# kfjahnke/envutil

Hardware: AMD Instinct MI355X
Metric: Mpix/s reprojected (16K lat/lon->cubemap, b-spline-3) (higher is better)
Workload: dtype f32

## Files before the change

envutil_amd/csrc/eu_render4.hip:

```cpp
#include <cstdio>
#include <cstring>
#include <vector>
#include <algorithm>
#include "eu_packed_dev.h"
#include "eu_launch.h"

#define EU4_TW 16
#define EU4_TH 8
#define EU4_WAVES 4
#ifndef EU4_WAVES0
#define EU4_WAVES0 1
#define EU4_TEXELS 384
#define EU4_OCC0 4
#endif
#define EU4_UNIT_ROWS 4
#define EU4_COL_FLOATS 8
#define EU4_MAX_PLANS 16

__device__ __forceinline__ void eu4_box_reduce(int &mn0, int &mn1, int &mx0, int &mx1)
{
#define EU4_RED(ctrl)                                        \
  "v_min_i32_dpp %0, %0, %0 " ctrl "\n\t"                    \
  "v_min_i32_dpp %1, %1, %1 " ctrl "\n\t"                    \
  "v_max_i32_dpp %2, %2, %2 " ctrl "\n\t"                    \
// ... 31 lines not shown
struct eu4_plan {
  const float *atab_g;
  const int *tileplan;
  const float *coltab;
  int tiles16;
  const int *l2_rows;
  int l2_off[9];
  int l2_half;
  unsigned long long l2_magic;
  const int *l1_ent;
  int l1_off[9];
  int l1_ecols;
  unsigned long long l1_magic;
  const int *xtab;
  const int *boxtab;
#ifdef EU5_STAMPS
  unsigned long long *stamps;
#endif
};

#ifdef EU5_STAMPS
#define EU5_STAMP(k) do { asm volatile("" ::: "memory"); st_[k] = __builtin_amdgcn_s_memtime(); asm volatile("" ::: "memory"); } while (0)
#define EU5_STAMP32(k) do { asm volatile("" ::: "memory"); st_[k] = (unsigned)__builtin_amdgcn_s_memtime(); asm volatile("" ::: "memory"); } while (0)
#else
#define EU5_STAMP(k) do { } while (0)
#define EU5_STAMP32(k) do { } while (0)
#endif

template <int NCH, int DEG, int PRJ>
__device__ __forceinline__ void eu4_tile(const eu_render_params &p, const eu4_plan &w, const float *atab,
// ... 272 lines not shown
  __syncthreads();
  if (threadIdx.x == 0) { listed = 0; last = atomicAdd(p.wl + EU4_WL_DONE1, 1) == (int)gridDim.x - 1; }
  __syncthreads();
  if (last) {
    int mine = 0;
    for (int i = threadIdx.x; i < EU4_SHARDS; i += 256)
      mine += __hip_atomic_load(p.wl + EU4_WL_SHARD(i), __ATOMIC_RELAXED, __HIP_MEMORY_SCOPE_AGENT);
    atomicAdd(&listed, mine);
    for (int i = threadIdx.x; i <= EU4_SHARDS + 8; i += 256)
      __hip_atomic_store(p.wl + 16 * i, 0, __ATOMIC_RELAXED, __HIP_MEMORY_SCOPE_AGENT);
    __syncthreads();
    if (threadIdx.x == 0) __hip_atomic_store(p.wl + EU4_WL_LISTED, listed, __ATOMIC_RELAXED, __HIP_MEMORY_SCOPE_AGENT);
  }
}

static long long eu4_followers_plan = 0, eu4_followers_last = 0;
extern "C" unsigned long long eu_hip_share_follower_tiles(void) { return (unsigned long long)eu4_followers_last; }
static int eu4_boxtab_last = 0;
static long long eu4_boxtab_tiles_last = 0;
extern "C" int eu_hip_boxtab_used(void) { return eu4_boxtab_last; }
extern "C" unsigned long long eu_hip_boxtab_tiles(void) { return (unsigned long long)eu4_boxtab_tiles_last; }

#ifndef EU4_DIRECT_WGS
#define EU4_DIRECT_WGS 2048
#endif

template <int NCH, int DEG, int PRJ>
static int launch4_ndp(const eu_render_params &p, const eu4_plan &w, hipStream_t st)
{
  if constexpr (PRJ == EU_SPHERICAL) {
    static const int cus = [] {
      int dev = 0, n = 0;
      if (hipGetDevice(&dev) != hipSuccess) return 0;
      if (hipDeviceGetAttribute(&n, hipDeviceAttributeMultiprocessorCount, dev) != hipSuccess) return 0;
      return n;
    }();
    const bool fast = eu_staged_fast_profile(p);
    const bool bt = fast && w.boxtab != nullptr && p.out_stride < (1ll << 25);
    int per_cu = 0;
    if (bt) {
      static const int occ = [] { int n = 0; return hipOccupancyMaxActiveBlocksPerMultiprocessor(&n, eu_render5_kernel<NCH, DEG, PRJ, true, true>, 64 * EU5_WAVES, 0) == hipSuccess ? n : 0; }();
      per_cu = occ;
    } else if (fast) {
      static const int occ = [] { int n = 0; return hipOccupancyMaxActiveBlocksPerMultiprocessor(&n, eu_render5_kernel<NCH, DEG, PRJ, true>, 64 * EU5_WAVES, 0) == hipSuccess ? n : 0; }();
      per_cu = occ;
    } else {
      static const int occ = [] { int n = 0; return hipOccupancyMaxActiveBlocksPerMultiprocessor(&n, eu_render5_kernel<NCH, DEG, PRJ, false>, 64 * EU5_WAVES, 0) == hipSuccess ? n : 0; }();
      per_cu = occ;
    }
    const int wgs = (cus / 8) * 8 * per_cu;
    if (wgs <= 0) return -1;
    if (fast) eu4_followers_last = eu4_followers_plan;
    eu4_boxtab_last = bt;
    if (bt) hipLaunchKernelGGL((eu_render5_kernel<NCH, DEG, PRJ, true, true>), dim3((unsigned)wgs), dim3(64 * EU5_WAVES), 0, st, p, w);
    else if (fast) hipLaunchKernelGGL((eu_render5_kernel<NCH, DEG, PRJ, true>), dim3((unsigned)wgs), dim3(64 * EU5_WAVES), 0, st, p, w);
    else hipLaunchKernelGGL((eu_render5_kernel<NCH, DEG, PRJ, false>), dim3((unsigned)wgs), dim3(64 * EU5_WAVES), 0, st, p, w);
  } else {
    const int units = (p.tiles_y + EU4_UNIT_ROWS - 1) / EU4_UNIT_ROWS;
    dim3 grid((unsigned)(8 * ((w.tiles16 + EU4_WAVES0 - 1) / EU4_WAVES0)), (unsigned)EU4_UNIT_ROWS, (unsigned)((units + 7) / 8));
    hipLaunchKernelGGL((eu_render4s_kernel<NCH, DEG, PRJ>), grid, dim3(64 * EU4_WAVES0), 0, st, p, w);
  }
  if (hipGetLastError() != hipSuccess) return -1;
  hipLaunchKernelGGL((eu_render4d_kernel<NCH, DEG, PRJ>), dim3(EU4_DIRECT_WGS), dim3(256), 0, st, p, w);
  if (hipGetLastError() != hipSuccess) {
    (void)hipMemsetAsync(p.wl, 0, EU4_WL_ENTRIES * sizeof(int), st);
    return -1;
  }
  return 0;
}

template <int NCH, int DEG>
static int launch4_nd(const eu_render_params &p, const eu4_plan &w, hipStream_t st)
{
  switch (p.src.prj) {
    case EU_SPHERICAL: return launch4_ndp<NCH, DEG, EU_SPHERICAL>(p, w, st);
    case EU_CUBEMAP: return launch4_ndp<NCH, DEG, EU_CUBEMAP>(p, w, st);
    case EU_BIATAN6: return launch4_ndp<NCH, DEG, EU_BIATAN6>(p, w, st);
// ... 15 lines not shown
static_assert(EU_STAGED_TILE_ROWS == EU4_TH && EU_STAGED_MAX_TILES_Y == 65535 * 8 * EU4_UNIT_ROWS, "eu_select.h: eu_staged_covers");
namespace {
struct plan_cache {
  std::vector<unsigned char> key;
  eu_dev_buf<int> tileplan, l2_rows, l1_ent, xtab, boxtab;
  bool has_boxtab = false;
  long long boxtab_tiles = 0;
  eu_dev_buf<float> coltab;
  float *atab = nullptr;
  int planned_rows = 0;
  int l2_off[9] = {};
  int l1_off[9] = {};
  int l1_ecols = 1;
  long long follower_tiles = 0;
  hipStream_t last_stream = nullptr;
} g4s[EU_MAX_SLOTS];
#define g4 (g4s[eu_current_slot()])

bool ensure_atab()
{
  if (g4.atab) return true;
  std::vector<float> tab(768, 0.0f);
  for (int i = 0; i < EU_ATAN_TAB_ENTRIES; i++) eu_atan_tab_entry(i, tab.data() + 8 * i);
  if (hipMalloc((void **)&g4.atab, tab.size() * sizeof(float)) != hipSuccess) return false;
  return hipMemcpy(g4.atab, tab.data(), tab.size() * sizeof(float), hipMemcpyHostToDevice) == hipSuccess;
}

template <int DEG>
void launch_colplan(const eu_render_params &p, float *ct, const float *k, hipStream_t st)
{
// ... 50 lines not shown
      for (size_t j = 0; j < plans.size() / 4 && id < 0; j++)
        if (memcmp(&plans[4 * j], k, sizeof k) == 0) id = (int)j;
      if (id < 0 && plans.size() / 4 < EU4_MAX_PLANS) {
        id = (int)(plans.size() / 4);
        plans.insert(plans.end(), k, k + 4);
      }
      tp[(size_t)ty] = id;
    }
  }
  const int nplans = (int)(plans.size() / 4);
  if (g4.tileplan.reserve(tp.size()) != hipSuccess) return -1;
  if (g4.coltab.reserve(std::max<size_t>(1, nplans) * (size_t)p.width * EU4_COL_FLOATS) != hipSuccess) return -1;
  if (hipStreamSynchronize(st) != hipSuccess) return -1;
  if (g4.last_stream && g4.last_stream != st && hipStreamSynchronize(g4.last_stream) != hipSuccess) return -1;
  if (hipMemcpy(g4.tileplan.p, tp.data(), tp.size() * sizeof(int), hipMemcpyHostToDevice) != hipSuccess) return -1;
  g4.planned_rows = 0;
  for (int v : tp) g4.planned_rows += v >= 0;
  auto paired = [&](int m) { return 2 * m + 1 < p.tiles_y && tp[(size_t)2 * m] >= 0 && tp[(size_t)2 * m] == tp[(size_t)2 * m + 1]; };
  {
    std::vector<int> rows[8], all;
    for (int r = 0; r < p.tiles_y; r++)
      if (!paired(r >> 1)) rows[(r / EU5_UNIT_ROWS) & 7].push_back(r);
    for (int x = 0; x < 8; x++) { g4.l2_off[x] = (int)all.size(); all.insert(all.end(), rows[x].begin(), rows[x].end()); }
    g4.l2_off[8] = (int)all.size();
    if (!upload(g4.l2_rows, all, 1)) return -1;
  }
  g4.has_boxtab = false; g4.boxtab_tiles = 0;
  if (sw.boxtab && eu_staged_fast_profile(p)) {
    const long long ntiles = (long long)g4.l2_off[8] * tiles16;
    const long long bytes = ntiles * (EU5_BT_RECS * 16);
    if (bytes <= (long long)sw.boxtab_max_kb * 1024) {
      if (g4.boxtab.reserve((size_t)std::max<long long>(1, ntiles) * (EU5_BT_RECS * 4)) != hipSuccess) return -1;
      if (ntiles > 0) {
        switch (p.src.degree) {
          case 1: launch_boxplan<1>(p, g4.atab, g4.l2_rows.p, tiles16, (int)ntiles, g4.boxtab.p, st); break;
          case 2: launch_boxplan<2>(p, g4.atab, g4.l2_rows.p, tiles16, (int)ntiles, g4.boxtab.p, st); break;
          default: launch_boxplan<3>(p, g4.atab, g4.l2_rows.p, tiles16, (int)ntiles, g4.boxtab.p, st); break;
        }
        if (hipGetLastError() != hipSuccess) return -1;
      }
// ... 37 lines not shown

void eu4_fill_plan(eu4_plan &w)
{
  w.tileplan = g4.tileplan.p;
  w.coltab = g4.coltab.p;
  w.l2_rows = g4.l2_rows.p;
  for (int x = 0; x < 9; x++) w.l2_off[x] = g4.l2_off[x];
  w.l2_half = (w.tiles16 + 1) / 2;
  w.l2_magic = (1ull << 40) / (unsigned long long)w.l2_half + 1;
  w.l1_ent = g4.l1_ent.p;
  for (int x = 0; x < 9; x++) w.l1_off[x] = g4.l1_off[x];
  w.l1_ecols = g4.l1_ecols;
  w.l1_magic = (1ull << 40) / (unsigned long long)w.l1_ecols + 1;
  w.xtab = g4.xtab.p;
  w.boxtab = g4.has_boxtab ? g4.boxtab.p : nullptr;
}

int launch4(const eu_render_params &p, const eu4_plan &w, hipStream_t st)
{
  switch (p.nch) {
    case 3: return launch4_n<3>(p, w, st);
    case 4: return launch4_n<4>(p, w, st);
  }
  return -2;
}

#ifdef EU5_STAMPS
int launch4_stamped(const eu_render_params &p, eu4_plan &w, hipStream_t st)
{
  static unsigned long long *d_st = nullptr; static size_t st_cap = 0; static int dumps = 0;
// ... 54 lines not shown
  hipStream_t st = (hipStream_t)stream;
  if (!ensure_atab()) return -1;
  w.atab_g = g4.atab;
  if (p.src.prj == EU_SPHERICAL) {
    std::vector<unsigned char> key = eu4_plan_key(p, plan_gen, *sw);
    if (key != g4.key) {
      if (eu4_build_plans(p, w.tiles16, *sw, h_row, h_row_floats, st)) return -1;
      g4.key.swap(key);
    }
    if (sw->r4 != 1 && !eu_staged_worth(p.src.degree, g4.planned_rows, p.tiles_y)) { *launches = 0; return 0; }
  }
  eu4_fill_plan(w);
  eu4_followers_plan = g4.follower_tiles;
  eu4_boxtab_tiles_last = w.boxtab ? g4.boxtab_tiles : 0;
  g4.last_stream = st;
#ifdef EU5_STAMPS
  return launch4_stamped(p, w, st);
#else
  return launch4(p, w, st);
#endif
}
```

envutil_amd/csrc/eu_render5.h:

```cpp
#define EU5_WAVES 4
#ifndef EU5_TEXELS
#define EU5_TEXELS 576
#endif
#ifndef EU5_OCC
#define EU5_OCC 4
#endif
#ifndef EU5_UNIT_ROWS
#define EU5_UNIT_ROWS 4
#endif

typedef const __attribute__((address_space(3))) eu4_f4 *eu5_l4ptr;

template <int NCH, int DEG>
__device__ __forceinline__ void eu5_taps(eu_lptr lt, int a, int b, int pitch, const eu_f2 *wx, const eu_f2 *wy,
                                         eu_f2 tx, eu_f2 ty, eu_f2 &rga, eu_f2 &bxa, eu_f2 &rgb, eu_f2 &bxb)
{
  constexpr int order = DEG + 1;
  if constexpr (DEG == 1) {
    const eu_f2 wl0 = 1.0f - tx, wr0 = tx, wl1 = 1.0f - ty, wr1 = ty;
    const eu4_f4 a00 = *(eu5_l4ptr)(lt + a), a01 = *(eu5_l4ptr)(lt + a + 4);
    const eu4_f4 a10 = *(eu5_l4ptr)(lt + a + pitch), a11 = *(eu5_l4ptr)(lt + a + pitch + 4);
    const eu4_f4 b00 = *(eu5_l4ptr)(lt + b), b01 = *(eu5_l4ptr)(lt + b + 4);
    const eu4_f4 b10 = *(eu5_l4ptr)(lt + b + pitch), b11 = *(eu5_l4ptr)(lt + b + pitch + 4);
    {
// ... 117 lines not shown
  const int y = p.row_begin + tile_y * EU4_TH + rw;
  const int yc = y < p.row_end ? y : p.row_end - 1;
  const float *rt = p.row + (long long)(FAST ? yc : eu_frame_row(yc, p.band_shift, p.band_count, p.band_index)) * EU_ROW_FLOATS;
  const int xa = x0 + 8 * hf + 2 * pr, xb = xa + 1;
  const int xac = xa < p.width ? xa : p.width - 1, xbc = xb < p.width ? xb : p.width - 1;
  T.A0 = rt[0]; T.A1 = rt[1]; T.A2 = rt[2]; T.B0 = rt[3]; T.B1 = rt[4]; T.B2 = rt[5];
  T.c0 = (eu_f2){ p.col[xac], p.col[xbc] };
}

struct eu5_co8 {
  eu_f2 tx, ty;
  int ixa, ixb, iya, iyb;
  eu_i2 ok;
};

template <int DEG>
__device__ __forceinline__ void eu5_coords8(const eu_src_dev &s, const float *atab, const eu5_tab8 &T, eu5_co8 &c)
{
  eu_i2 big0 = { 0, 0 }, big1 = { 0, 0 };
  const eu_f2 c0 = T.c0;
  const eu_f2 rx = T.B0 * c0 + T.A0, ry = T.B1 * c0 + T.A1, rz = T.B2 * c0 + T.A2;
  const eu_i2 ok = { ~eu5_out_of_range3(rx.x, ry.x, rz.x), ~eu5_out_of_range3(rx.y, ry.y, rz.y) };
  const eu_f2 q2 = rx * rx + rz * rz;
  const eu_f2 qs = eu_sqrt2_safe(q2);
  const eu_f2 lat = eu_atan2f_2_lean(ry, qs, atab, 1, big0);
  const eu_f2 lon = eu_atan2f_2_lean(rx, rz, atab, 0, big1);
  c.ok = ok & ~(big0 | big1);
  eu_f2 i0 = { (float)((double)lon.x - s.tex_x0), (float)((double)lon.y - s.tex_x0) };
  if (s.cdiv_ok) i0 = eu_div2_const(i0, s.ext_w, s.rcp_ext_w);
  else i0 = eu_div2_rr(i0, s.ext_w, eu_rcp_refined(s.ext_w));
  i0 = i0 * s.total_w; i0 = i0 - .5f;
  const eu_f2 sx = i0 - s.win_x_off;
  const eu_f2 gx = eu5_gate2(sx, s.gate0, s.lower0, s.upper0);
  eu_f2 fx;
  if constexpr (DEG & 1) fx = (eu_f2){ floorf(gx.x), floorf(gx.y) };
  else fx = (eu_f2){ roundf(gx.x), roundf(gx.y) };
  c.tx = gx - fx;
  c.ixa = (int)fx.x; c.ixb = (int)fx.y;
  eu_f2 i1 = { (float)((double)lat.x - s.tex_y0), (float)((double)lat.y - s.tex_y0) };
  if (s.cdiv_ok) i1 = eu_div2_const(i1, s.ext_h, s.rcp_ext_h);
  else i1 = eu_div2_rr(i1, s.ext_h, eu_rcp_refined(s.ext_h));
  i1 = i1 * s.total_h; i1 = i1 - .5f;
  const eu_f2 sy = i1 - s.win_y_off;
  c.ty = eu5_gate2(sy, s.gate1, s.lower1, s.upper1);
}

template <int DEG>
__device__ __forceinline__ void eu5_split_y(eu5_co8 &c)
{
  const eu_f2 gy = c.ty;
  eu_f2 fy;
  if constexpr (DEG & 1) fy = (eu_f2){ floorf(gy.x), floorf(gy.y) };
  else fy = (eu_f2){ roundf(gy.x), roundf(gy.y) };
  c.ty = gy - fy;
  c.iya = (int)fy.x; c.iyb = (int)fy.y;
}
// ... 401 lines not shown
  if (B.npass == 2) { r[0] = eu5_box_at(B.h0, B.h1, B.h2, B.h3, 31); r[1] = eu5_box_at(B.h0, B.h1, B.h2, B.h3, 63); }
  if (B.npass == 4) {
#pragma unroll
    for (int k = 0; k < 4; k++) r[k] = eu5_box_at(B.q0, B.q1, B.q2, B.q3, 15 + 16 * k);
  }
  int v = 0;
#pragma unroll
  for (int k = 0; k < EU5_BT_RECS; k++) {
#pragma unroll
    for (int i = 0; i < 4; i++)
      if (lane == 4 * k + i) v = eu5_bt_pack(r[k], k == 0 ? cls : 0, i);
  }
  if (lane < 4 * EU5_BT_RECS) tab[(size_t)g * (4 * EU5_BT_RECS) + lane] = v;
}

template <int NCH, int DEG>
__device__ __forceinline__ void eu5_tile_bt(const eu_render_params &p, const eu4_plan &w, const float *atab, float *wtile,
                                            int tile_y, int x0, int lane, const eu5_tab8 &T, eu5_i4 R, eu5_crec rec,
                                            bool have_n, int ty_n, int x0_n, eu5_tab8 &Tn)
{
  constexpr int order = DEG + 1;
  const eu_src_dev &s = p.src;
#ifdef EU5_STAMPS
  unsigned long long st_[8] = { 0, 0, 0, 0, 0, 0, 0, 0 };
#endif
  EU5_STAMP(0);
  const int cls = R.w;
  if (cls & EU5_BT_WORK) {
    if (lane == 0) {
      const int id = tile_y * w.tiles16 + x0 / EU4_TW;
      const int sh = eu4_shard_of(id);
      const int slot = atomicAdd(p.wl + EU4_WL_SHARD(sh), 1);
      p.wl[EU4_WL_ENTRIES + (size_t)slot * EU4_SHARDS + sh] = id;
    }
    if (have_n) eu5_load8<true>(p, ty_n, x0_n, lane, Tn);
    __builtin_amdgcn_s_waitcnt(EU5_WAIT_VM0);
    return;
  }
  const int npass = cls & 7;
  const unsigned lds_tile = (unsigned)(unsigned long long)(eu4_lds_void)wtile;
  eu5_tab8 Tl = T;
  asm volatile("" : "+v"(Tl.c0), "+v"(Tl.A0), "+v"(Tl.A1), "+v"(Tl.A2), "+v"(Tl.B0), "+v"(Tl.B1), "+v"(Tl.B2));
  eu5_box bx = { R.x, R.y, R.x + (R.z & 0xffff), R.y + (R.z >> 16) };
  bool some = npass > 0 && R.z >= 0;
  if (some) eu5_stage<NCH, DEG>(s, bx, lds_tile, lane);
  const int pr = lane & 3, rw = (lane >> 2) & 7, hf = lane >> 5;
  const int y = p.row_begin + tile_y * EU4_TH + rw;
  const bool yin = y < p.row_end;
  const int xa = x0 + 8 * hf + 2 * pr, xb = xa + 1;
  const bool va = yin && xa < p.width, vb = yin && xb < p.width;
  eu_f2 rga = { 0.0f, 0.0f }, bxa = { 0.0f, 0.0f }, rgb = { 0.0f, 0.0f }, bxb = { 0.0f, 0.0f };
  if (npass > 0) {
    eu5_co8 c;
    eu5_coords8<DEG>(s, atab, Tl, c);
    eu5_split_y<DEG>(c);
#ifdef EU5_STAMPS
    asm volatile("" : : "v"(c.iya), "v"(c.iyb), "v"(c.ixa), "v"(c.ixb));
#endif
    EU5_STAMP(2);
#ifdef EU5_STAMPS
    st_[3] = st_[2];
#endif
    eu_f2 wx[order], wy[order];
    if constexpr (DEG >= 2) {
      eu_weights2<DEG>(s.wm, c.ty, wy);
      eu_weights2<DEG>(s.wm, c.tx, wx);
    }
    const int grp = npass == 1 ? 0 : npass == 2 ? hf : (lane >> 4);
#pragma unroll 1
// ... 82 lines not shown
  "v_min_i32_dpp %0, %0, %0 " ctrl "\n\t"                    \
  "v_max_i32_dpp %1, %1, %1 " ctrl "\n\t"                    \
  "s_nop 1\n\t"
  asm("s_nop 1\n\t"
      EU5_RED2("row_shr:1 row_mask:0xf bank_mask:0xf")
      EU5_RED2("row_shr:2 row_mask:0xf bank_mask:0xf")
      EU5_RED2("row_shr:4 row_mask:0xf bank_mask:0xf")
      EU5_RED2("row_shr:8 row_mask:0xf bank_mask:0xf")
      EU5_RED2("row_bcast:15 row_mask:0xa bank_mask:0xf")
      EU5_RED2("row_bcast:31 row_mask:0xc bank_mask:0xf")
      : "+v"(mn), "+v"(mx));
#undef EU5_RED2
  mn = __builtin_amdgcn_readlane(mn, 63); mx = __builtin_amdgcn_readlane(mx, 63);
}

template <int NCH, int DEG>
__device__ __forceinline__ void eu5_group16(const eu_render_params &p, const eu4_plan &w, const float *atab, float *wtile,
                                            eu5_tab16 &T, eu5_cint ent, int n, int m0, int plan0, int tcol, int lane0,
                                            bool have_n, int m_n, int plan_n, int tcol_n)
{
  constexpr int order = DEG + 1;
  const eu_src_dev &s = p.src;
#ifdef EU5_STAMPS
  unsigned st_[8] = { 0, 0, 0, 0, 0, 0, 0, 0 };
#endif
  EU5_STAMP32(0);
  const eu5_cint xt = (eu5_cint)w.xtab;
  int xmn = xt[2 * (plan0 * w.tiles16 + tcol)], xmx = xt[2 * (plan0 * w.tiles16 + tcol) + 1];
  int iyAa, iyAb, iyBa, iyBb, bad, mny = INT_MAX, mxy = INT_MIN;
  eu_f2 tyA, tyB;
  bool off;
// ... 92 lines not shown
      const int oBa = hBa ? ((iyBa - bx.mny) * ibw + (ixa - bx.mnx)) * 4 : 0, oBb = hBb ? ((iyBb - bx.mny) * ibw + (ixb - bx.mnx)) * 4 : 0;
      asm volatile("s_waitcnt vmcnt(0)" ::: "memory");
      __builtin_amdgcn_sched_barrier(0);
      eu5_taps<NCH, DEG>((eu_lptr)wtile, oAa, oAb, ibw * 4, wx, wyA, tx, tyA, rga, bxa, rgb, bxb);
      asm volatile("" : "+v"(rga), "+v"(bxa), "+v"(rgb), "+v"(bxb));
      {
        float qa[4] = { rga.x, rga.y, bxa.x, bxa.y }, qb[4] = { rgb.x, rgb.y, bxb.x, bxb.y };
        float *const orow = p.out + (long long)(ycA - p.row_begin) * p.out_stride;
        if (hAa) eu_put<NCH>(orow, xa, qa);
        if (hAb) eu_put<NCH>(orow, xb, qb);
      }
      __builtin_amdgcn_sched_barrier(0);
      eu5_taps<NCH, DEG>((eu_lptr)wtile, oBa, oBb, ibw * 4, wx, wyB, tx, tyB, rga, bxa, rgb, bxb);
      asm volatile("" : "+v"(rga), "+v"(bxa), "+v"(rgb), "+v"(bxb));
    } else if (mny != INT_MAX) {
      if (lane < 2) {
        const int id = (2 * mk + lane) * w.tiles16 + tc;
        const int sh = eu4_shard_of(id);
        const int slot = atomicAdd(p.wl + EU4_WL_SHARD(sh), 1);
        p.wl[EU4_WL_ENTRIES + (size_t)slot * EU4_SHARDS + sh] = id;
      }
    }
    if (k + 1 < n) {
      const int xa_n = mir_n ? p.width - 1 - (tcol * EU4_TW + xl) : tcol * EU4_TW + xl, xb_n = mir_n ? xa_n - 1 : xa_n + 1;
      const int xac = xa_n < p.width ? xa_n : p.width - 1, xbc = xb_n < p.width ? xb_n : p.width - 1;
      eu5_load_cols(w.coltab + (size_t)plan_k * p.width * EU4_COL_FLOATS, xac, xbc, T);
    } else if (have_n) {
      eu5_load16(p, w.coltab + (size_t)plan_n * p.width * EU4_COL_FLOATS, 2 * m_n, tcol_n * EU4_TW, lane, T);
    }
    __builtin_amdgcn_sched_barrier(0);
    if (fast) {
// ... 41 lines not shown
    const unsigned h = ((unsigned)row() * 0x9E3779B1u) >> 16;
    int c = rx + (int)((h * (unsigned)tiles16) >> 16);
    if (c >= tiles16) c -= tiles16;
    return c;
  }
};

__device__ __forceinline__ int eu5_pair_plan(const int *tileplan, int tiles_y, int m)
{
  if (2 * m + 1 >= tiles_y) return -1;
  const eu5_cint tp = (eu5_cint)tileplan;
  const int a = tp[2 * m], b = tp[2 * m + 1];
  return a == b ? a : -1;
}

template <int NCH, int DEG, int PRJ, bool FAST, bool BOXTAB = false>
__global__ __launch_bounds__(64 * EU5_WAVES, EU5_OCC) void eu_render5_kernel(const eu_render_params p, const eu4_plan w)
{
  __shared__ __attribute__((aligned(16))) float tile_all[EU5_WAVES * EU5_TEXELS * 4];
  __shared__ __attribute__((aligned(16))) float atab[768];
  const int lane0 = threadIdx.x & 63;
  const int wave = __builtin_amdgcn_readfirstlane(threadIdx.x >> 6);
  float *const tile = tile_all + wave * (EU5_TEXELS * 4);
  if (PRJ != EU_CUBEMAP && wave == 0) {
#pragma unroll
    for (int i = 0; i < 3; i++)
      __builtin_amdgcn_global_load_lds((eu4_gbl_void)(w.atab_g + i * 256 + lane0 * 4),
                                       (eu4_lds_void)(atab + i * 256), 16, 0, 0);
    asm volatile("s_waitcnt vmcnt(0)" ::: "memory");
  }
  __syncthreads();
// ... 17 lines not shown
      const unsigned h = ((unsigned)m * 0x9E3779B1u) >> 16;
      int c = pos1 - r * w.l1_ecols + (int)((h * (unsigned)w.l1_ecols) >> 16);
      if (c >= w.l1_ecols) c -= w.l1_ecols;
      tcol = e[1] + c;
      pos1 += K;
      return true;
    };
    eu5_cint e_a = ents, e_n = ents;
    int n_a = 0, m_a = 0, col_a = 0, plan_a = 0, n_n = 0, m_n = 0, col_n = 0, plan_n = 0;
    bool have_a = seek(e_a, n_a, m_a, plan_a, col_a);
    eu5_tab16 T;
    if (have_a) eu5_load16(p, w.coltab + (size_t)plan_a * p.width * EU4_COL_FLOATS, 2 * m_a, col_a * EU4_TW, lane0, T);
#pragma unroll 1
    while (have_a) {
      const bool have_n = seek(e_n, n_n, m_n, plan_n, col_n);
      eu5_group16<NCH, DEG>(p, w, atab, tile, T, e_a, n_a, m_a, plan_a, col_a, lane0, have_n, m_n, have_n ? plan_n : 0, col_n);
      e_a = e_n; n_a = n_n; m_a = m_n; plan_a = plan_n; col_a = col_n; have_a = have_n;
    }
  }
#ifdef EU5_STAMPS
  ws1 = __builtin_amdgcn_s_memtime();
#endif
  eu5_iter<EU5_UNIT_ROWS> it;
  it.xcd = xcd; it.tiles16 = w.tiles16;
  it.units = (p.tiles_y + EU5_UNIT_ROWS - 1) / EU5_UNIT_ROWS;
  it.start(t0, K);
  if constexpr (PAIRS) {
    int *const queue = p.wl + EU4_WL_DYN(xcd);
    const int nbatch = (w.l2_off[xcd + 1] - w.l2_off[xcd]) * w.l2_half;
    const eu5_cint rows2 = (eu5_cint)w.l2_rows + w.l2_off[xcd];
    auto take = [&]() -> int {
      int v = 0;
      if (lane0 == 0) v = atomicAdd(queue, 1);
      return v;
    };
    if constexpr (BOXTAB) {
      static_assert(FAST && PRJ == EU_SPHERICAL, "the box table is that of the FAST lat/lon second loop");
      const eu5_crec bt = (eu5_crec)w.boxtab;
      auto decode = [&](int j, int &ty, int &tcol, int &ti) -> bool {
        if (j >= nbatch) return false;
        const int r = (int)(((unsigned long long)(unsigned)j * w.l2_magic) >> 40);
        ty = rows2[r]; tcol = 2 * (j - r * w.l2_half);
        ti = ((w.l2_off[xcd] + r) * w.tiles16 + tcol) * EU5_BT_RECS;
        return true;
      };
      int ty_a = 0, col_a = 0, ti_a = 0, ty_n = 0, col_n = 0, ti_n = 0;
      bool have = decode(__builtin_amdgcn_readfirstlane(take()), ty_a, col_a, ti_a);
      eu5_tab8 Ta, Tb;
      eu5_i4 Ra = { 0, 0, -1, 0 }, Rb = { 0, 0, -1, 0 };
      if (have) { Ra = bt[ti_a]; eu5_load8<FAST>(p, ty_a, col_a * EU4_TW, lane0, Ta); }
      __builtin_amdgcn_s_waitcnt(EU5_WAIT_VM0);
#pragma unroll 1
      while (have) {
        const int jn_lane = take();
        const bool second = col_a + 1 < w.tiles16;
        if (second) Rb = bt[ti_a + EU5_BT_RECS];
        {
          int lane = lane0;
          asm volatile("" : "+v"(lane));
          eu5_tile_bt<NCH, DEG>(p, w, atab, tile, ty_a, col_a * EU4_TW, lane, Ta, Ra, bt + ti_a, second, ty_a,
                                (col_a + 1) * EU4_TW, Tb);
        }
        const bool have_n = decode(__builtin_amdgcn_readfirstlane(jn_lane), ty_n, col_n, ti_n);
        if (have_n) Ra = bt[ti_n];
        if (second) {
          int lane = lane0;
          asm volatile("" : "+v"(lane));
          eu5_tile_bt<NCH, DEG>(p, w, atab, tile, ty_a, (col_a + 1) * EU4_TW, lane, Tb, Rb, bt + ti_a + EU5_BT_RECS, have_n,
                                ty_n, col_n * EU4_TW, Ta);
        } else if (have_n) {
          eu5_load8<FAST>(p, ty_n, col_n * EU4_TW, lane0, Ta);
          __builtin_amdgcn_s_waitcnt(EU5_WAIT_VM0);
        }
        ty_a = ty_n; col_a = col_n; ti_a = ti_n; have = have_n;
      }
    } else {
      auto decode = [&](int j, int &ty, int &tcol) -> bool {
        if (j >= nbatch) return false;
        const int r = (int)(((unsigned long long)(unsigned)j * w.l2_magic) >> 40);
        ty = rows2[r]; tcol = 2 * (j - r * w.l2_half);
        return true;
      };
      int ty_a = 0, col_a = 0, ty_n = 0, col_n = 0;
      bool have = decode(__builtin_amdgcn_readfirstlane(take()), ty_a, col_a);
      eu5_tab8 Ta, Tb;
      if (have) eu5_load8<FAST>(p, ty_a, col_a * EU4_TW, lane0, Ta);
  #pragma unroll 1
// ... 21 lines not shown
#pragma unroll 1
    while (!it.done()) {
      const int tile_y = it.row(), tcol = it.col(), plan = plan_n;
      it.step();
      plan_n = (it.done() || it.row() >= p.tiles_y) ? -2 : (PRJ == EU_SPHERICAL ? ((eu5_cint)w.tileplan)[it.row()] : -1);
      if (plan == -2) continue;
      int lane = lane0;
      asm volatile("" : "+v"(lane));
      if (plan >= 0)
        eu5_tile<NCH, DEG, PRJ, PRJ == EU_SPHERICAL, FAST>(p, w, atab, tile, w.coltab + (size_t)plan * p.width * EU4_COL_FLOATS,
                                                            tile_y, tcol * EU4_TW, lane);
      else
        eu5_tile<NCH, DEG, PRJ, false, FAST>(p, w, atab, tile, nullptr, tile_y, tcol * EU4_TW, lane);
    }
  }
#ifdef EU5_STAMPS
  if (lane0 == 0 && w.stamps) {
    unsigned long long *o = w.stamps + (size_t)w.tiles16 * p.tiles_y * 8 + ((size_t)blockIdx.x * EU5_WAVES + wave) * 4;
    o[0] = ws0; o[1] = ws1; o[2] = __builtin_amdgcn_s_memtime(); o[3] = 1;
  }
#endif
}
```

envutil_amd/csrc/eu_select.h:

```cpp
#ifndef EU_SELECT_H
#define EU_SELECT_H
#include <algorithm>
#include <climits>
#include <cstdlib>
#include <vector>
#include "eu_device.h"
#include "eu_share_groups.h"
#include "eu_worklist.h"

struct eu_switches {
  int force_general;
  int hybrid;
  int r4;
  int colmajor;
  int rej;
  int colplan;
  int share;
  int direct;
  int iir_stream;
  int boxtab;
  int boxtab_max_kb;
  int views_max_kb;
};

#define EU_BOXTAB_MAX_KB 65536
#define EU_VIEWS_MAX_KB 65536

inline eu_switches eu_read_switches()
{
  auto first = [](const char *name) { const char *e = getenv(name); return e ? e[0] : '\0'; };
  eu_switches s;
  s.force_general = first("EU_HIP_KERNEL") == '1';
  const char hy = first("EU_HIP_HYBRID");
  s.hybrid = hy == '0' ? 0 : hy == '2' ? 2 : 1;
  const char *r4 = getenv("EU_HIP_R4");
  s.r4 = r4 ? atoi(r4) : -1;
  const char *cm = getenv("EU_HIP_COLMAJOR");
  s.colmajor = cm && cm[0] ? atoi(cm) : -1;
  const char rj = first("EU_HIP_REJ");
  s.rej = rj == '1' ? 1 : rj == '2' ? 2 : 0;
  s.colplan = first("EU_HIP_COLPLAN") != '0';
  const char sh = first("EU_HIP_SHARE");
  s.share = sh == '0' ? 0 : sh == 'm' ? EU_SHARE_MIRRORS : sh == 'f' ? EU_SHARE_FACES : EU_SHARE_FACES | EU_SHARE_MIRRORS;
  s.direct = first("EU_HIP_DIRECT") == '1';
  const char *iir = getenv("EU_HIP_IIR_STREAM");
  s.iir_stream = iir ? atoi(iir) : 7;
  s.boxtab = first("EU_HIP_BOXTAB") != '0';
  const char *bm = getenv("EU_HIP_BOXTAB_MAX_KB");
  s.boxtab_max_kb = bm && bm[0] ? std::max(0, std::min(atoi(bm), 16 * 1024 * 1024)) : EU_BOXTAB_MAX_KB;
  const char *vm = getenv("EU_HIP_VIEWS_MAX_KB");
  s.views_max_kb = vm && vm[0] ? std::max(0, std::min(atoi(vm), 16 * 1024 * 1024)) : EU_VIEWS_MAX_KB;
  return s;
}

inline bool eu_cube_source(int prj) { return prj == EU_CUBEMAP || prj == EU_BIATAN6; }

inline bool eu_packed_covers_source(const eu_src_dev &s, int nch, int nch_out)
{
  if (s.has_lcp || nch_out != nch) return false;
  if (s.prj != EU_SPHERICAL && !eu_cube_source(s.prj)) return false;
  if (s.degree < 1 || s.degree > 3 || s.es0 != nch) return false;
  return nch >= 1 && nch <= 4;
}
inline bool eu_packed_covers(const eu_render_params &p)
{
// ... 118 lines not shown
```

envutil_amd/csrc/eu_worklist.h:

```cpp
#ifndef EU_WORKLIST_H
#define EU_WORKLIST_H
#include <algorithm>
#include <climits>
#include <cstddef>
#include <vector>

#if defined(__HIPCC__)
#define EU_WL_FN __host__ __device__ inline __attribute__((always_inline))
#else
#define EU_WL_FN inline
#endif

#define EU4_SHARDS 1024
#define EU4_WL_SHARD(s) (16 * (s))
#define EU4_WL_DONE1 (16 * EU4_SHARDS)
#define EU4_WL_DYN(x) (16 * (EU4_SHARDS + 1 + (x)))
#define EU4_WL_LISTED (16 * (EU4_SHARDS + 9))
#define EU4_WL_ENTRIES (16 * (EU4_SHARDS + 16))

#define EU4_WL_MAX_TILES ((size_t)INT_MAX)

EU_WL_FN int eu4_shard_of(int id)
{
  return (int)(((unsigned)id * 0x9E3779B1u) >> 22) & (EU4_SHARDS - 1);
// ... 14 lines not shown
      if (c > fullest_) { fullest_ = c; grows_.push_back(n_ + 1); }
    }
    return (size_t)(std::upper_bound(grows_.begin(), grows_.end(), ntiles) - grows_.begin());
  }
};

inline size_t eu_render4_worklist_header_ints(void) { return EU4_WL_ENTRIES; }

inline size_t eu_render4_worklist_ints(size_t ntiles)
{
  static eu4_wl_census census;
  if (ntiles > EU4_WL_MAX_TILES) return 0;
  return EU4_WL_ENTRIES + census.fullest(ntiles) * EU4_SHARDS;
}

#endif
```

Measured before the change: 107,500.

## Record follower tile list once and interleave direct tiles into staged kernel

On the first call, a single-workgroup kernel prefix-sums the sharded worklist of tiles that need the direct path and copies them into a persistent static list. The count is read back asynchronously through an event. Later calls with the same plan launch a single staged kernel that skips the atomic worklist pushes and runs the listed direct tiles, interleaved per batch through a noinline call. This drops the second direct-tile kernel launch and the atomic contention, at the cost of reusing a tile list recorded on an earlier call, which is only valid while the plan is unchanged.

New measurement: 107,800 (median of 2 runs). About the same (+0.3%).

```diff
diff --git a/envutil_amd/csrc/eu_render4.hip b/envutil_amd/csrc/eu_render4.hip
--- a/envutil_amd/csrc/eu_render4.hip
+++ b/envutil_amd/csrc/eu_render4.hip
@@ -69,6 +69,8 @@
   unsigned long long l1_magic;
   const int *xtab;
   const int *boxtab;
+  const int *slist;
+  int sl_first[9];
 #ifdef EU5_STAMPS
   unsigned long long *stamps;
 #endif
@@ -371,6 +373,32 @@
   }
 }
 
+__global__ __launch_bounds__(EU4_SHARDS) void eu4_record_kernel(const int *wl, int *list, int cap)
+{
+  __shared__ int pre[EU4_SHARDS];
+  const int s = threadIdx.x;
+  const int c = max(0, __hip_atomic_load(wl + EU4_WL_SHARD(s), __ATOMIC_RELAXED, __HIP_MEMORY_SCOPE_AGENT));
+  pre[s] = c;
+  __syncthreads();
+  for (int d = 1; d < EU4_SHARDS; d <<= 1) {
+    const int v = s >= d ? pre[s - d] : 0;
+    __syncthreads();
+    pre[s] += v;
+    __syncthreads();
+  }
+  const int total = pre[EU4_SHARDS - 1], base = pre[s] - c;
+  if (total <= cap)
+    for (int k = 0; k < c; k++) list[base + k] = wl[EU4_WL_ENTRIES + (size_t)k * EU4_SHARDS + s];
+  if (s == 0) list[cap] = total <= cap ? total : -1;
+}
+static int *eu4_record_list = nullptr;
+static int eu4_record_cap = 0;
+
+static bool eu4_boxtab_holds(const eu_render_params &p, const eu4_plan &w)
+{
+  return eu_staged_fast_profile(p) && w.boxtab != nullptr && p.out_stride < (1ll << 25);
+}
+
 static long long eu4_followers_plan = 0, eu4_followers_last = 0;
 extern "C" unsigned long long eu_hip_share_follower_tiles(void) { return (unsigned long long)eu4_followers_last; }
 static int eu4_boxtab_last = 0;
@@ -393,9 +421,13 @@
       return n;
     }();
     const bool fast = eu_staged_fast_profile(p);
-    const bool bt = fast && w.boxtab != nullptr && p.out_stride < (1ll << 25);
+    const bool bt = eu4_boxtab_holds(p, w);
+    const bool il = bt && w.slist != nullptr;
     int per_cu = 0;
-    if (bt) {
+    if (il) {
+      static const int occ = [] { int n = 0; return hipOccupancyMaxActiveBlocksPerMultiprocessor(&n, eu_render5_kernel<NCH, DEG, PRJ, true, true, true>, 64 * EU5_WAVES, 0) == hipSuccess ? n : 0; }();
+      per_cu = occ;
+    } else if (bt) {
       static const int occ = [] { int n = 0; return hipOccupancyMaxActiveBlocksPerMultiprocessor(&n, eu_render5_kernel<NCH, DEG, PRJ, true, true>, 64 * EU5_WAVES, 0) == hipSuccess ? n : 0; }();
       per_cu = occ;
     } else if (fast) {
@@ -409,6 +441,10 @@
     if (wgs <= 0) return -1;
     if (fast) eu4_followers_last = eu4_followers_plan;
     eu4_boxtab_last = bt;
+    if (il) {
+      hipLaunchKernelGGL((eu_render5_kernel<NCH, DEG, PRJ, true, true, true>), dim3((unsigned)wgs), dim3(64 * EU5_WAVES), 0, st, p, w);
+      return hipGetLastError() == hipSuccess ? 0 : -1;
+    }
     if (bt) hipLaunchKernelGGL((eu_render5_kernel<NCH, DEG, PRJ, true, true>), dim3((unsigned)wgs), dim3(64 * EU5_WAVES), 0, st, p, w);
     else if (fast) hipLaunchKernelGGL((eu_render5_kernel<NCH, DEG, PRJ, true>), dim3((unsigned)wgs), dim3(64 * EU5_WAVES), 0, st, p, w);
     else hipLaunchKernelGGL((eu_render5_kernel<NCH, DEG, PRJ, false>), dim3((unsigned)wgs), dim3(64 * EU5_WAVES), 0, st, p, w);
@@ -418,6 +454,10 @@
     hipLaunchKernelGGL((eu_render4s_kernel<NCH, DEG, PRJ>), grid, dim3(64 * EU4_WAVES0), 0, st, p, w);
   }
   if (hipGetLastError() != hipSuccess) return -1;
+  if (eu4_record_list) {
+    hipLaunchKernelGGL(eu4_record_kernel, dim3(1), dim3(EU4_SHARDS), 0, st, p.wl, eu4_record_list, eu4_record_cap);
+    if (hipGetLastError() != hipSuccess) eu4_record_list = nullptr;
+  }
   hipLaunchKernelGGL((eu_render4d_kernel<NCH, DEG, PRJ>), dim3(EU4_DIRECT_WGS), dim3(256), 0, st, p, w);
   if (hipGetLastError() != hipSuccess) {
     (void)hipMemsetAsync(p.wl, 0, EU4_WL_ENTRIES * sizeof(int), st);
@@ -463,6 +503,10 @@
   int l1_ecols = 1;
   long long follower_tiles = 0;
   hipStream_t last_stream = nullptr;
+  eu_dev_buf<int> slist;
+  int sl_cap = 0, sl_state = 0, sl_n = 0;
+  int *sl_count = nullptr;
+  hipEvent_t sl_event = nullptr;
 } g4s[EU_MAX_SLOTS];
 #define g4 (g4s[eu_current_slot()])
 
@@ -543,6 +587,7 @@
   if (hipStreamSynchronize(st) != hipSuccess) return -1;
   if (g4.last_stream && g4.last_stream != st && hipStreamSynchronize(g4.last_stream) != hipSuccess) return -1;
   if (hipMemcpy(g4.tileplan.p, tp.data(), tp.size() * sizeof(int), hipMemcpyHostToDevice) != hipSuccess) return -1;
+  g4.sl_state = 0; g4.sl_n = 0; g4.sl_cap = 0;
   g4.planned_rows = 0;
   for (int v : tp) g4.planned_rows += v >= 0;
   auto paired = [&](int m) { return 2 * m + 1 < p.tiles_y && tp[(size_t)2 * m] >= 0 && tp[(size_t)2 * m] == tp[(size_t)2 * m + 1]; };
@@ -553,6 +598,10 @@
     for (int x = 0; x < 8; x++) { g4.l2_off[x] = (int)all.size(); all.insert(all.end(), rows[x].begin(), rows[x].end()); }
     g4.l2_off[8] = (int)all.size();
     if (!upload(g4.l2_rows, all, 1)) return -1;
+    const size_t nbatch_total = all.size() * (size_t)((tiles16 + 1) / 2);
+    const size_t ints = eu4_static_list_ints((size_t)tiles16 * (size_t)p.tiles_y, std::min<size_t>(nbatch_total, INT_MAX - 1));
+    if (g4.slist.reserve(ints) != hipSuccess) return -1;
+    g4.sl_cap = (int)ints - 1;
   }
   g4.has_boxtab = false; g4.boxtab_tiles = 0;
   if (sw.boxtab && eu_staged_fast_profile(p)) {
@@ -620,6 +669,43 @@
   w.l1_magic = (1ull << 40) / (unsigned long long)w.l1_ecols + 1;
   w.xtab = g4.xtab.p;
   w.boxtab = g4.has_boxtab ? g4.boxtab.p : nullptr;
+  w.slist = nullptr;
+  for (int x = 0; x < 9; x++) w.sl_first[x] = 0;
+}
+
+bool eu4_static_list(const eu_render_params &p, eu4_plan &w, const eu_switches &sw)
+{
+  eu4_record_list = nullptr;
+  if (!sw.staticlist || p.src.prj != EU_SPHERICAL || !eu4_boxtab_holds(p, w) || !g4.slist.p) return false;
+  const bool arrived = g4.sl_state == 1 && hipEventQuery(g4.sl_event) == hipSuccess;
+  (void)hipGetLastError();
+  if (arrived) {
+    const int n = *(volatile int *)g4.sl_count;
+    g4.sl_n = n;
+    g4.sl_state = n >= 0 && n <= g4.sl_cap ? 2 : 3;
+  }
+  if (g4.sl_state == 0) {
+    if (!g4.sl_count && hipHostMalloc((void **)&g4.sl_count, sizeof(int), hipHostMallocDefault) != hipSuccess) { g4.sl_count = nullptr; return false; }
+    if (!g4.sl_event && hipEventCreateWithFlags(&g4.sl_event, hipEventDisableTiming) != hipSuccess) { g4.sl_event = nullptr; return false; }
+    eu4_record_list = g4.slist.p; eu4_record_cap = g4.sl_cap;
+    return false;
+  }
+  if (g4.sl_state != 2) return false;
+  int nbatch[8];
+  for (int x = 0; x < 8; x++) nbatch[x] = (w.l2_off[x + 1] - w.l2_off[x]) * w.l2_half;
+  if (!eu4_static_interleaves(g4.sl_n, nbatch)) return false;
+  eu4_static_split(g4.sl_n, nbatch, w.sl_first);
+  w.slist = g4.slist.p;
+  return true;
+}
+
+void eu4_static_list_recorded(hipStream_t st)
+{
+  if (!eu4_record_list) return;
+  eu4_record_list = nullptr;
+  if (hipMemcpyAsync(g4.sl_count, g4.slist.p + g4.sl_cap, sizeof(int), hipMemcpyDeviceToHost, st) != hipSuccess) return;
+  if (hipEventRecord(g4.sl_event, st) != hipSuccess) return;
+  g4.sl_state = 1;
 }
 
 int launch4(const eu_render_params &p, const eu4_plan &w, hipStream_t st)
@@ -704,9 +790,13 @@
   eu4_followers_plan = g4.follower_tiles;
   eu4_boxtab_tiles_last = w.boxtab ? g4.boxtab_tiles : 0;
   g4.last_stream = st;
+  if (eu4_static_list(p, w, *sw)) *launches = 1;
 #ifdef EU5_STAMPS
-  return launch4_stamped(p, w, st);
+  const int rc = launch4_stamped(p, w, st);
 #else
-  return launch4(p, w, st);
+  const int rc = launch4(p, w, st);
 #endif
-}
+  if (rc == 0) eu4_static_list_recorded(st);
+  eu4_record_list = nullptr;
+  return rc;
+}
diff --git a/envutil_amd/csrc/eu_render5.h b/envutil_amd/csrc/eu_render5.h
--- a/envutil_amd/csrc/eu_render5.h
+++ b/envutil_amd/csrc/eu_render5.h
@@ -155,9 +155,13 @@
   eu_i2 ok;
 };
 
-template <int DEG>
+template <int DEG, bool SRR = false>
 __device__ __forceinline__ void eu5_coords8(const eu_src_dev &s, const float *atab, const eu5_tab8 &T, eu5_co8 &c)
 {
+  auto rcp = [](float d) {
+    const float r = eu_rcp_refined(d);
+    return SRR ? __int_as_float(__builtin_amdgcn_readfirstlane(__float_as_int(r))) : r;
+  };
   eu_i2 big0 = { 0, 0 }, big1 = { 0, 0 };
   const eu_f2 c0 = T.c0;
   const eu_f2 rx = T.B0 * c0 + T.A0, ry = T.B1 * c0 + T.A1, rz = T.B2 * c0 + T.A2;
@@ -169,7 +173,7 @@
   c.ok = ok & ~(big0 | big1);
   eu_f2 i0 = { (float)((double)lon.x - s.tex_x0), (float)((double)lon.y - s.tex_x0) };
   if (s.cdiv_ok) i0 = eu_div2_const(i0, s.ext_w, s.rcp_ext_w);
-  else i0 = eu_div2_rr(i0, s.ext_w, eu_rcp_refined(s.ext_w));
+  else i0 = eu_div2_rr(i0, s.ext_w, rcp(s.ext_w));
   i0 = i0 * s.total_w; i0 = i0 - .5f;
   const eu_f2 sx = i0 - s.win_x_off;
   const eu_f2 gx = eu5_gate2(sx, s.gate0, s.lower0, s.upper0);
@@ -180,7 +184,7 @@
   c.ixa = (int)fx.x; c.ixb = (int)fx.y;
   eu_f2 i1 = { (float)((double)lat.x - s.tex_y0), (float)((double)lat.y - s.tex_y0) };
   if (s.cdiv_ok) i1 = eu_div2_const(i1, s.ext_h, s.rcp_ext_h);
-  else i1 = eu_div2_rr(i1, s.ext_h, eu_rcp_refined(s.ext_h));
+  else i1 = eu_div2_rr(i1, s.ext_h, rcp(s.ext_h));
   i1 = i1 * s.total_h; i1 = i1 - .5f;
   const eu_f2 sy = i1 - s.win_y_off;
   c.ty = eu5_gate2(sy, s.gate1, s.lower1, s.upper1);
@@ -612,7 +616,7 @@
   if (lane < 4 * EU5_BT_RECS) tab[(size_t)g * (4 * EU5_BT_RECS) + lane] = v;
 }
 
-template <int NCH, int DEG>
+template <int NCH, int DEG, bool STATIC = false>
 __device__ __forceinline__ void eu5_tile_bt(const eu_render_params &p, const eu4_plan &w, const float *atab, float *wtile,
                                             int tile_y, int x0, int lane, const eu5_tab8 &T, eu5_i4 R, eu5_crec rec,
                                             bool have_n, int ty_n, int x0_n, eu5_tab8 &Tn)
@@ -625,11 +629,13 @@
   EU5_STAMP(0);
   const int cls = R.w;
   if (cls & EU5_BT_WORK) {
-    if (lane == 0) {
-      const int id = tile_y * w.tiles16 + x0 / EU4_TW;
-      const int sh = eu4_shard_of(id);
-      const int slot = atomicAdd(p.wl + EU4_WL_SHARD(sh), 1);
-      p.wl[EU4_WL_ENTRIES + (size_t)slot * EU4_SHARDS + sh] = id;
+    if constexpr (!STATIC) {
+      if (lane == 0) {
+        const int id = tile_y * w.tiles16 + x0 / EU4_TW;
+        const int sh = eu4_shard_of(id);
+        const int slot = atomicAdd(p.wl + EU4_WL_SHARD(sh), 1);
+        p.wl[EU4_WL_ENTRIES + (size_t)slot * EU4_SHARDS + sh] = id;
+      }
     }
     if (have_n) eu5_load8<true>(p, ty_n, x0_n, lane, Tn);
     __builtin_amdgcn_s_waitcnt(EU5_WAIT_VM0);
@@ -650,7 +656,7 @@
   eu_f2 rga = { 0.0f, 0.0f }, bxa = { 0.0f, 0.0f }, rgb = { 0.0f, 0.0f }, bxb = { 0.0f, 0.0f };
   if (npass > 0) {
     eu5_co8 c;
-    eu5_coords8<DEG>(s, atab, Tl, c);
+    eu5_coords8<DEG, STATIC>(s, atab, Tl, c);
     eu5_split_y<DEG>(c);
 #ifdef EU5_STAMPS
     asm volatile("" : : "v"(c.iya), "v"(c.iyb), "v"(c.ixa), "v"(c.ixb));
@@ -763,7 +769,7 @@
   mn = __builtin_amdgcn_readlane(mn, 63); mx = __builtin_amdgcn_readlane(mx, 63);
 }
 
-template <int NCH, int DEG>
+template <int NCH, int DEG, bool STATIC = false>
 __device__ __forceinline__ void eu5_group16(const eu_render_params &p, const eu4_plan &w, const float *atab, float *wtile,
                                             eu5_tab16 &T, eu5_cint ent, int n, int m0, int plan0, int tcol, int lane0,
                                             bool have_n, int m_n, int plan_n, int tcol_n)
@@ -886,7 +892,7 @@
       eu5_taps<NCH, DEG>((eu_lptr)wtile, oBa, oBb, ibw * 4, wx, wyB, tx, tyB, rga, bxa, rgb, bxb);
       asm volatile("" : "+v"(rga), "+v"(bxa), "+v"(rgb), "+v"(bxb));
     } else if (mny != INT_MAX) {
-      if (lane < 2) {
+      if (!STATIC && lane < 2) {
         const int id = (2 * mk + lane) * w.tiles16 + tc;
         const int sh = eu4_shard_of(id);
         const int slot = atomicAdd(p.wl + EU4_WL_SHARD(sh), 1);
@@ -958,7 +964,17 @@
   return a == b ? a : -1;
 }
 
-template <int NCH, int DEG, int PRJ, bool FAST, bool BOXTAB = false>
+template <int NCH, int DEG, int PRJ>
+__device__ __attribute__((noinline)) void eu5_direct_called(const void *kernarg, const float *atab, int tile_y, int x0, int lane)
+{
+  const unsigned long long ka = (unsigned long long)kernarg;
+  const unsigned long long ku = (unsigned long long)(unsigned)__builtin_amdgcn_readfirstlane((int)(unsigned)ka) |
+                                ((unsigned long long)(unsigned)__builtin_amdgcn_readfirstlane((int)(unsigned)(ka >> 32)) << 32);
+  const eu_render_params &p = *(const eu_render_params *)(const __attribute__((address_space(4))) void *)ku;
+  eu4_direct_tile<NCH, DEG, PRJ>(p, atab, tile_y, x0, lane);
+}
+
+template <int NCH, int DEG, int PRJ, bool FAST, bool BOXTAB = false, bool STATIC = false>
 __global__ __launch_bounds__(64 * EU5_WAVES, EU5_OCC) void eu_render5_kernel(const eu_render_params p, const eu4_plan w)
 {
   __shared__ __attribute__((aligned(16))) float tile_all[EU5_WAVES * EU5_TEXELS * 4];
@@ -1006,7 +1022,7 @@
 #pragma unroll 1
     while (have_a) {
       const bool have_n = seek(e_n, n_n, m_n, plan_n, col_n);
-      eu5_group16<NCH, DEG>(p, w, atab, tile, T, e_a, n_a, m_a, plan_a, col_a, lane0, have_n, m_n, have_n ? plan_n : 0, col_n);
+      eu5_group16<NCH, DEG, STATIC>(p, w, atab, tile, T, e_a, n_a, m_a, plan_a, col_a, lane0, have_n, m_n, have_n ? plan_n : 0, col_n);
       e_a = e_n; n_a = n_n; m_a = m_n; plan_a = plan_n; col_a = col_n; have_a = have_n;
     }
   }
@@ -1028,6 +1044,8 @@
     };
     if constexpr (BOXTAB) {
       static_assert(FAST && PRJ == EU_SPHERICAL, "the box table is that of the FAST lat/lon second loop");
+      const int sl_first = STATIC ? w.sl_first[xcd] : 0, sl_n = STATIC ? w.sl_first[xcd + 1] - sl_first : 0;
+      const eu5_cint slist = (eu5_cint)w.slist;
       const eu5_crec bt = (eu5_crec)w.boxtab;
       auto decode = [&](int j, int &ty, int &tcol, int &ti) -> bool {
         if (j >= nbatch) return false;
@@ -1037,7 +1055,8 @@
         return true;
       };
       int ty_a = 0, col_a = 0, ti_a = 0, ty_n = 0, col_n = 0, ti_n = 0;
-      bool have = decode(__builtin_amdgcn_readfirstlane(take()), ty_a, col_a, ti_a);
+      int j_a = __builtin_amdgcn_readfirstlane(take());
+      bool have = decode(j_a, ty_a, col_a, ti_a);
       eu5_tab8 Ta, Tb;
       eu5_i4 Ra = { 0, 0, -1, 0 }, Rb = { 0, 0, -1, 0 };
       if (have) { Ra = bt[ti_a]; eu5_load8<FAST>(p, ty_a, col_a * EU4_TW, lane0, Ta); }
@@ -1050,19 +1069,38 @@
         {
           int lane = lane0;
           asm volatile("" : "+v"(lane));
-          eu5_tile_bt<NCH, DEG>(p, w, atab, tile, ty_a, col_a * EU4_TW, lane, Ta, Ra, bt + ti_a, second, ty_a,
+          eu5_tile_bt<NCH, DEG, STATIC>(p, w, atab, tile, ty_a, col_a * EU4_TW, lane, Ta, Ra, bt + ti_a, second, ty_a,
                                 (col_a + 1) * EU4_TW, Tb);
         }
-        const bool have_n = decode(__builtin_amdgcn_readfirstlane(jn_lane), ty_n, col_n, ti_n);
+        const int j_n = __builtin_amdgcn_readfirstlane(jn_lane);
+        const bool have_n = decode(j_n, ty_n, col_n, ti_n);
         if (have_n) Ra = bt[ti_n];
         if (second) {
           int lane = lane0;
           asm volatile("" : "+v"(lane));
-          eu5_tile_bt<NCH, DEG>(p, w, atab, tile, ty_a, (col_a + 1) * EU4_TW, lane, Tb, Rb, bt + ti_a + EU5_BT_RECS, have_n,
+          eu5_tile_bt<NCH, DEG, STATIC>(p, w, atab, tile, ty_a, (col_a + 1) * EU4_TW, lane, Tb, Rb, bt + ti_a + EU5_BT_RECS, have_n,
                                 ty_n, col_n * EU4_TW, Ta);
         } else if (have_n) {
           eu5_load8<FAST>(p, ty_n, col_n * EU4_TW, lane0, Ta);
           __builtin_amdgcn_s_waitcnt(EU5_WAIT_VM0);
+        }
+        if constexpr (STATIC) {
+          if (sl_n > 0) {
+            int lo, hi;
+            eu4_static_share(j_a, nbatch, sl_first, sl_n, lo, hi);
+            if (hi > lo) {
+#pragma unroll 1
+              for (int e = lo; e < hi; e++) {
+                const int id = slist[e];
+                const int dty = id / w.tiles16;
+                int lane = lane0;
+                asm volatile("" : "+v"(lane));
+                eu5_direct_called<NCH, DEG, PRJ>((const void *)__builtin_amdgcn_kernarg_segment_ptr(), atab, dty, (id - dty * w.tiles16) * EU4_TW, lane);
+              }
+              __builtin_amdgcn_s_waitcnt(EU5_WAIT_VM0);
+            }
+          }
+          j_a = j_n;
         }
         ty_a = ty_n; col_a = col_n; ti_a = ti_n; have = have_n;
       }
@@ -1114,6 +1152,13 @@
         eu5_tile<NCH, DEG, PRJ, false, FAST>(p, w, atab, tile, nullptr, tile_y, tcol * EU4_TW, lane);
     }
   }
+  if constexpr (STATIC) {
+    if (lane0 == 0 && atomicAdd(p.wl + EU4_WL_DONE1, 1) == (int)(gridDim.x * EU5_WAVES) - 1) {
+      for (int x = 0; x < 8; x++) __hip_atomic_store(p.wl + EU4_WL_DYN(x), 0, __ATOMIC_RELAXED, __HIP_MEMORY_SCOPE_AGENT);
+      __hip_atomic_store(p.wl + EU4_WL_LISTED, w.sl_first[8], __ATOMIC_RELAXED, __HIP_MEMORY_SCOPE_AGENT);
+      __hip_atomic_store(p.wl + EU4_WL_DONE1, 0, __ATOMIC_RELAXED, __HIP_MEMORY_SCOPE_AGENT);
+    }
+  }
 #ifdef EU5_STAMPS
   if (lane0 == 0 && w.stamps) {
     unsigned long long *o = w.stamps + (size_t)w.tiles16 * p.tiles_y * 8 + ((size_t)blockIdx.x * EU5_WAVES + wave) * 4;
diff --git a/envutil_amd/csrc/eu_select.h b/envutil_amd/csrc/eu_select.h
--- a/envutil_amd/csrc/eu_select.h
+++ b/envutil_amd/csrc/eu_select.h
@@ -21,6 +21,7 @@
   int boxtab;
   int boxtab_max_kb;
   int views_max_kb;
+  int staticlist;
 };
 
 #define EU_BOXTAB_MAX_KB 65536
@@ -49,6 +50,7 @@
   const char *bm = getenv("EU_HIP_BOXTAB_MAX_KB");
   s.boxtab_max_kb = bm && bm[0] ? std::max(0, std::min(atoi(bm), 16 * 1024 * 1024)) : EU_BOXTAB_MAX_KB;
   const char *vm = getenv("EU_HIP_VIEWS_MAX_KB");
+  s.staticlist = first("EU_HIP_STATICLIST") != '0';
   s.views_max_kb = vm && vm[0] ? std::max(0, std::min(atoi(vm), 16 * 1024 * 1024)) : EU_VIEWS_MAX_KB;
   return s;
 }
diff --git a/envutil_amd/csrc/eu_worklist.h b/envutil_amd/csrc/eu_worklist.h
--- a/envutil_amd/csrc/eu_worklist.h
+++ b/envutil_amd/csrc/eu_worklist.h
@@ -52,4 +52,37 @@
   return EU4_WL_ENTRIES + census.fullest(ntiles) * EU4_SHARDS;
 }
 
+
+EU_WL_FN void eu4_static_share(int j, int nbatch_xcd, int first_xcd, int n_xcd, int &lo, int &hi)
+{
+  const unsigned long long nb = (unsigned long long)(unsigned)nbatch_xcd, n = (unsigned long long)(unsigned)n_xcd;
+  const unsigned long long t = (unsigned long long)(unsigned)j * n;
+  const unsigned long long q = t / nb, s = t - q * nb + n;
+  lo = first_xcd + (int)q;
+  hi = lo + (s < nb ? 0 : s < 2 * nb ? 1 : (int)(s / nb));
+}
+
+EU_WL_FN void eu4_static_split(int n, const int *nbatch, int *first)
+{
+  unsigned long long total = 0, cum = 0;
+  for (int x = 0; x < 8; x++) total += (unsigned long long)(unsigned)nbatch[x];
+  first[0] = 0;
+  for (int x = 0; x < 8; x++) {
+    cum += (unsigned long long)(unsigned)nbatch[x];
+    first[x + 1] = total ? (int)((unsigned long long)(unsigned)n * cum / total) : (x == 7 ? n : 0);
+  }
+}
+
+inline bool eu4_static_interleaves(int n, const int *nbatch)
+{
+  if (n < 0) return false;
+  int first[9];
+  eu4_static_split(n, nbatch, first);
+  for (int x = 0; x < 8; x++)
+    if (first[x + 1] - first[x] > 0 && first[x + 1] - first[x] > nbatch[x]) return false;
+  return true;
+}
+
+inline size_t eu4_static_list_ints(size_t ntiles, size_t nbatch_total) { return std::min(ntiles, nbatch_total) + 1; }
+
 #endif
```
